# una-auxme/MeshGraphNets.jl

Measured on AMD Instinct MI355X. Metric: processor-step edges/s, higher is better.
Workload: dtype f32; 1 GPU; M-1M jittered-grid triangulation 1000x1000: N=1000000 nodes, E=5992002 directed edges, L=128, hidden_layers=2, 15 processor steps per bench step, fp32 storage, fp16x2 split MFMA (every fp32 operand = two fp16 pieces after a power-of-two scaling per weight chunk / per activation row, three exact piece products per fp32 product on v_mfma_f32_32x32x16_f16), fp32 accumulate; held to the fp32 tolerance; partition=single partition, edge_order=engine re-sorts by receiver once per trajectory (mgn_set_graph)

## Files before the change

meshgraphnets.jl_amd/csrc/kernels.h:

```cpp
#pragma once
#include <hip/hip_runtime.h>
#include <stdint.h>

namespace mgn {

constexpr int TILE = 32;
constexpr int MAX_CHUNKS = 9;

enum { T_B1 = 0, T_B2, T_B3, T_GAMMA, T_BETA, T_BQ, T_LN, T_COUNT };

struct GenMlp {
    const float* chunk[4];
    const float* tabs;
    int32_t nmid;
    int32_t use;
};

struct EdgeArgs {
    const int32_t* snd;
    const int32_t* rcv;
    int64_t E;
    int32_t ntiles;
    const float* P;
    const float* Q;
    float* Elat;
    const float* ElatSrc;
    float* AGG;
    float* CARRY;
    const float* chunk[MAX_CHUNKS];
    const float* chunk_t[MAX_CHUNKS];
    const float* tabs;
    int32_t stagger;
    int32_t tile0;
    unsigned long long* stamps;
    GenMlp gen;
    int32_t c16;
    int32_t bf;
    const uint16_t* split[3];
    const uint16_t* split16[3];
    const uint16_t* splith[3];
    const uint16_t* split16h[3];
    float h2_s[3], h2_rs[3], h2_b2pos;
};

struct NodeArgs {
    int32_t n;
    int32_t ntiles;
    const int32_t* rowptr;
    float* V;
    const float* AGG;
    const float* CARRY;
    float* P;
    float* Q;
    const float* chunk[MAX_CHUNKS];
    const float* chunk_t[MAX_CHUNKS];
    const int32_t* rowptr2; const float* AGG2; const float* CARRY2; int64_t zero_row2;
    const float* tabs;
    int32_t mode;
    int32_t stagger;
    int64_t zero_row;
    int32_t tile0;
    GenMlp gen;
    int32_t c16;
    float* P2; float* Q2; const float* tabs2;
    int32_t bf;
    unsigned long long* stamps;
    const uint16_t* split[7];
    const uint16_t* split16[9];
    const uint16_t* splith[6];
    const uint16_t* split16h[9];
    float h2_s[9], h2_rs[9], h2_b2pos;
};

struct EncNodeArgs {
    int32_t n, ntiles;
    const int32_t* gid;
    const float* srcA; int32_t wa;
    const float* srcB; int32_t wb;
    const float* scale;
    const float* shift;
    const float* w1f;
    float* V; float* P; float* Q;
    const float* chunk[MAX_CHUNKS];
    const float* tabs;
    GenMlp gen;
    const uint16_t* splith[4];
    float h2_rs[4];
};

struct EncEdgeArgs {
    int64_t E; int32_t ntiles;
    const int64_t* gid;
    const float* ef; int32_t Fe;
    const float* scale; const float* shift;
    const float* w1f;
    float* Elat;
    const float* chunk[MAX_CHUNKS];
    const float* tabs;
    GenMlp gen;
    const uint16_t* splith[2];
    float h2_rs[2];
};

struct DecArgs {
    int32_t n, ntiles;
    const float* V;
    const float* w3f;
    const float* b3;
    int32_t O;
    const float* oscale; const float* oshift;
    const float* mask;
    const int32_t* gid;
    float* out;
    const float* chunk[MAX_CHUNKS];
    const float* tabs;
    GenMlp gen;
    const uint16_t* splith[2];
    float h2_rs[2];
};

struct BfEdgeArgs {
    const int32_t* snd; const int32_t* rcv; int64_t E; int32_t ntiles; int32_t tile0;
    const uint16_t* P; const uint16_t* Q;
    uint16_t* Elat; uint16_t* AGG;
    uint16_t* CARRY;
    const uint16_t* chunk[3];
    const float* tabs;
    unsigned long long* stamps;
};
struct BfNodeArgs {
    int32_t n, ntiles; const int32_t* rowptr;
    uint16_t* V; const uint16_t* AGG; const uint16_t* CARRY; uint16_t* P; uint16_t* Q;
    const uint16_t* chunk[7];
    const float* tabs;
    int64_t zero_row; int32_t tile0;
    const int32_t* rowptr2; const uint16_t* AGG2; const uint16_t* CARRY2; int64_t zero_row2;
};
hipError_t launch_edge_bf16(const BfEdgeArgs& a, hipStream_t s);
hipError_t launch_node_bf16(const BfNodeArgs& a, hipStream_t s);
hipError_t launch_project_bf16(const BfNodeArgs& a, hipStream_t s);
hipError_t launch_tile_f32_to_bf16(const float* src, uint16_t* dst, int64_t ntiles, hipStream_t s);
hipError_t launch_tile_bf16_to_f32(const uint16_t* src, float* dst, int64_t ntiles, hipStream_t s);
hipError_t launch_scatter_prows(const float* src, int src_stride , float* dst, int64_t row0, int64_t rows, int L, hipStream_t s);
hipError_t launch_scatter_prows16(const uint16_t* src, int src_stride , uint16_t* dst, int64_t row0, int64_t rows, hipStream_t s);
bool prows_blocked();
hipError_t launch_gather_rows16(const uint16_t* src, const int32_t* idx, uint16_t* dst, int64_t rows, int dst_stride , hipStream_t s);

struct LaunchCfg { int blocks; int threads; size_t lds; };
hipError_t launch_node_split_h(const NodeArgs& a, const LaunchCfg& lc, hipStream_t s);
hipError_t launch_project_split_h(const NodeArgs& a, const LaunchCfg& lc, hipStream_t s);
hipError_t launch_edge_ring_h(const EdgeArgs& a, const LaunchCfg& lc, hipStream_t s);
size_t edge_ring_h_lds();
int set_ringh_stream(int on);
int edge_ring_h_streamed();
hipError_t launch_edge_ring(const EdgeArgs& a, const LaunchCfg& lc, hipStream_t s);
hipError_t launch_node_split(const NodeArgs& a, const LaunchCfg& lc, hipStream_t s);
hipError_t launch_project_split(const NodeArgs& a, const LaunchCfg& lc, hipStream_t s);

struct LinComb {
    int n;
    float c[7];
    const float* k[7];
};
hipError_t launch_lincomb(float* out, const float* u, const LinComb& lc, float dt, int64_t n, hipStream_t s);
hipError_t launch_overwrite(float* x, const float* frame, const uint8_t* mask, int64_t N, int O, hipStream_t s);
int errnorm_partials();
hipError_t launch_errnorm(const float* u, const float* unew, const LinComb& lc, float dt, float atol, float rtol, int64_t n,
                          double* partial, hipStream_t s);
int save_error_blocks(int64_t rows);
hipError_t launch_save_error(const float* x, const float* gt, double* acc, double* part, int64_t N, int O, hipStream_t s);
struct EvalFinish {
    const double* acc;
    const double* part;
    int64_t N; int O, n_saves;
    const int32_t* gid;
    const int64_t* sel;
    int64_t n_val;
    float* mse_time;
    double* mse_save;
    double* vpart;
    int blocks, val_blocks, time_blocks;
};
hipError_t launch_eval_finish(EvalFinish f, hipStream_t s);

bool launch_is_small(int ntiles);
bool node_split_size(int ntiles);
bool launch_is_small_edge(int ntiles_e);
int coop16_enabled();
int set_c16_edge_tiles(int t);
bool ring_hs_default();
bool coop16_size(int ntiles_e, int ntiles_n, bool ring_hs = false);
int last_edge_kernel();
int last_node_kernel();
int set_fp32_split(int on);
int fp32_split_enabled();
int set_split_f16(int on);
int split_f16_enabled();
int set_c16_split(int on);
int c16_split_enabled();
int set_c16_row_tiles(int rt);
int set_kernel_path(int p);
int get_kernel_path();
int set_num_cus(int n);
int num_cus_override();
hipError_t launch_edge_step(int L, const EdgeArgs& a, hipStream_t s);
hipError_t launch_node_step(int L, const NodeArgs& a, hipStream_t s);
hipError_t launch_project(int L, const NodeArgs& a, hipStream_t s);
hipError_t launch_node_project_fused(int L, const NodeArgs& a, hipStream_t s, bool* launched);
hipError_t launch_node_ring_hs(const NodeArgs& a, const LaunchCfg& lc, hipStream_t s);
int node_ring_hs_enabled();
int set_node_ring_hs(int on);
hipError_t launch_enc_node(int L, const EncNodeArgs& a, hipStream_t s);
hipError_t launch_enc_edge(int L, const EncEdgeArgs& a, hipStream_t s);
hipError_t launch_decode(int L, const DecArgs& a, hipStream_t s);
hipError_t launch_gather_rows(const float* src, const int32_t* idx, float* dst, int64_t rows, int L, int dst_stride , hipStream_t s);
hipError_t launch_rows_to_tiles(const float* src, const int64_t* gid64, const int32_t* gid32, float* dst, int64_t rows, int L, hipStream_t s);
hipError_t launch_tiles_to_rows(const float* src, const int64_t* gid64, const int32_t* gid32, float* dst, int64_t rows, int L, hipStream_t s);
hipError_t launch_randn_rows(float* dst, const int64_t* gid64, const int32_t* gid32, int64_t rows, int L,
                             uint64_t seed, hipStream_t s);
int kernels_prow_block();
int split_prow_block();
int checksum_partials();
hipError_t launch_checksum(const float* src, int64_t n, double* partials, hipStream_t s);

}
```

meshgraphnets.jl_amd/csrc/mgn_api.cpp:

```cpp
#include <hip/hip_runtime.h>

#include <algorithm>
#include <cmath>
#include <cstdarg>
#include <cstdint>
#include <cstdio>
#include <cstdlib>
#include <cstring>
#include <ctime>
#include <string>
#include <sys/stat.h>
#include <unistd.h>
#include <vector>

#include "engine_internal.h"
#include "train.h"
#include "graph_dev.h"

using namespace mgn;


namespace {

thread_local std::string g_create_error;
// ... 2146 lines not shown
            if (!write_atomic(ack_of(rank), &rec.nonce, 8)) return fail(h, MGN_E_RCCL, "mgn_comm_init_file: cannot write %s", ack_of(rank).c_str());
            const double t_ack = mtime_of(ack_of(rank));
            for (;;) {
                uint64_t n = 0;
                if (read_exact(go, &n, 8) && mtime_of(go) >= t_ack) {
                    confirmed = n == rec.nonce;
                    break;
                }
                IdFile cur{};
                if (read_exact(base, &cur, sizeof cur) && cur.nonce != rec.nonce) break;
                if (waited > limit) return fail(h, MGN_E_RCCL, "mgn_comm_init_file: timed out waiting for rank 0 to confirm %s", path);
                nap20ms();
                waited += 0.02;
            }
            if (!confirmed) { nap20ms(); waited += 0.02; }
        }
    }
    const int rc = mgn_comm_init(h, rec.id, MGN_COMM_ID_BYTES, transport);
    if (rank == 0) {
        unlink(path);
        unlink(go.c_str());
        for (int r = 1; r < nranks; ++r) unlink(ack_of(r).c_str());
    }
    return rc;
} MGN_CATCH(h)

int mgn_comm_destroy(mgn_handle* h) try {
    if (!h) return MGN_E_ARG;
    if (!h->host_only) (void)hipStreamSynchronize(h->stream);
    delete h->comm;
    h->comm = nullptr;
    h->hx_ready = false;
    h->all_gid.clear();
    return MGN_OK;
} MGN_CATCH(h)

int mgn_comm_barrier(mgn_handle* h) try {
    if (!h) return MGN_E_ARG;
    if (int rc = need_comm(h, "mgn_comm_barrier")) return rc;
    COMMCHK(h, h->comm->barrier(h->stream));
    return MGN_OK;
} MGN_CATCH(h)

int mgn_comm_allreduce(mgn_handle* h, double* x, int32_t n, int32_t op) try {
    if (!h) return MGN_E_ARG;
    if (int rc = need_comm(h, "mgn_comm_allreduce")) return rc;
    if (!x || n < 0 || (op != 0 && op != 1)) return fail(h, MGN_E_ARG, "mgn_comm_allreduce: bad argument");
    COMMCHK(h, h->comm->allreduce_f64(x, n, op, h->stream));
    return MGN_OK;
} MGN_CATCH(h)

int mgn_halo_exchange(mgn_handle* h) try {
    if (int rc = need(h, false, true)) return rc;
    if (int rc = need_comm(h, "mgn_halo_exchange")) return rc;
    if (int rc = exchange_start(h)) return rc;
    return exchange_finish(h);
} MGN_CATCH(h)

int mgn_halo_exchange_host(mgn_handle* h, const float* own_rows, float* halo_rows, int32_t width) try {
    if (!h || !h->have_graph) return fail(h, MGN_E_STATE, "mgn_halo_exchange_host before mgn_set_graph");
    if (int rc = need_comm(h, "mgn_halo_exchange_host")) return rc;
    if (width < 1 || (!own_rows && h->g.n_own) || (!halo_rows && h->g.n_halo)) return fail(h, MGN_E_ARG, "mgn_halo_exchange_host: bad argument");
    const LocalGraph& g = h->g;
    const int P = h->cfg.nranks;
    const size_t rowb = (size_t)width * 4;
    std::vector<float> send(g.send_idx.size() * (size_t)width);
    for (size_t i = 0; i < g.send_idx.size(); ++i) memcpy(send.data() + i * width, own_rows + (size_t)g.send_idx[i] * width, rowb);
    std::vector<size_t> sb(P), so(P), rb(P), ro(P);
    size_t s0 = 0, r0 = 0;
    for (int q = 0; q < P; ++q) {
        sb[q] = (size_t)g.send_rows[q] * rowb; so[q] = s0; s0 += sb[q];
        rb[q] = (size_t)g.recv_rows[q] * rowb; ro[q] = r0; r0 += rb[q];
    }
    COMMCHK(h, h->comm->a2a_host(send.data(), sb.data(), so.data(), halo_rows, rb.data(), ro.data()));
    return MGN_OK;
} MGN_CATCH(h)

int mgn_debug_kernel_path(int path) { return set_kernel_path(path); }
int mgn_debug_c16_row_tiles(int rt) { return set_c16_row_tiles(rt); }
int mgn_debug_c16_edge_tiles(int t) { return set_c16_edge_tiles(t); }
int mgn_debug_fp32_split(int on) { return set_fp32_split(on); }
int mgn_debug_split_f16(int on) { return set_split_f16(on); }
int mgn_debug_ringh_stream(int on) { return set_ringh_stream(on); }
int mgn_debug_node_ring_hs(int on) { return set_node_ring_hs(on); }
int mgn_debug_num_cus(int n) { return set_num_cus(n); }
int mgn_debug_train_f16(int on) { return set_train_f16(on); }
long long mgn_debug_pack_check(mgn_handle* h) try {
    if (int rc = need(h, true, false)) return -rc;
    const int L = h->cfg.L;
    const size_t CH = (size_t)L * L;
    const float* p = h->params.data();
    long long bad = 0;
    std::vector<float> hf(3 * CH), df(3 * CH);
    std::vector<uint16_t> hb(3 * 16384), db(3 * 16384);
    for (const WPackJob& jb : h->wjobs) {
        const float* W = p + jb.src;
        if (jb.kind == 0) {
            const size_t n = (L == 128 ? 3 : 2) * CH;
            pack_chunk(hf.data(), W, jb.ldw, jb.kbase, L);
            pack_chunk_tmajor(hf.data() + CH, hf.data(), L);
            if (L == 128) pack_chunk16(hf.data() + 2 * CH, W, jb.ldw, jb.kbase);
            if (hipMemcpy(df.data(), h->wfrag.as<float>() + jb.off, n * 4, hipMemcpyDeviceToHost) != hipSuccess) return -MGN_E_HIP;
            for (size_t i = 0; i < n; ++i) bad += memcmp(&hf[i], &df[i], 4) != 0;
        } else if (jb.kind == 3) {
            pack_chunk_bf16(hb.data(), W, jb.ldw, jb.kbase);
            if (hipMemcpy(db.data(), h->wbf.as<uint16_t>() + jb.off, 16384 * 2, hipMemcpyDeviceToHost) != hipSuccess) return -MGN_E_HIP;
            for (size_t i = 0; i < 16384; ++i) bad += hb[i] != db[i];
        } else if (jb.kind == 4 || jb.kind == 5) {
            pack_chunk_split_h(hb.data(), W, jb.ldw, jb.kbase, jb.scale, jb.kind == 5);
            if (hipMemcpy(db.data(), h->wsp.as<uint16_t>() + jb.off, 2 * 16384 * 2, hipMemcpyDeviceToHost) != hipSuccess) return -MGN_E_HIP;
            for (size_t i = 0; i < 2 * 16384; ++i) bad += hb[i] != db[i];
        } else {
            pack_chunk_split(hb.data(), W, jb.ldw, jb.kbase, jb.kind == 2);
            if (hipMemcpy(db.data(), h->wsp.as<uint16_t>() + jb.off, 3 * 16384 * 2, hipMemcpyDeviceToHost) != hipSuccess) return -MGN_E_HIP;
            for (size_t i = 0; i < 3 * 16384; ++i) bad += hb[i] != db[i];
        }
    }
    return bad;
} catch (...) { return -MGN_E_OOM; }
int mgn_debug_c16_split(int on) { return set_c16_split(on); }
int mgn_debug_last_node_kernel(void) { return last_node_kernel(); }
int mgn_debug_last_edge_kernel(void) { return last_edge_kernel(); }
int mgn_debug_renumber(int mode) { const int old = g_renumber; g_renumber = mode; return old; }
int mgn_debug_renumbered(const mgn_handle* h) { return h && h->have_graph && h->g.renumbered ? 1 : 0; }

int mgn_debug_edge_stamps(mgn_handle* h, int32_t k, unsigned long long* out ) try {
    if (int rc = need(h, true, true)) return rc;
    const size_t n = 32768;
    HIPCHK(h, h->d_stamps.ensure(n * 8));
    HIPCHK(h, hipMemsetAsync(h->d_stamps.p, 0, n * 8, h->stream));
    if (int rc = mgn_proc_edge(h, k)) return rc;
    HIPCHK(h, hipMemcpyAsync(out, h->d_stamps.p, n * 8, hipMemcpyDeviceToHost, h->stream));
    HIPCHK(h, hipStreamSynchronize(h->stream));
    h->d_stamps.release();
    return MGN_OK;
} MGN_CATCH(h)

int mgn_debug_node_stamps(mgn_handle* h, int32_t k, unsigned long long* out ) try {
    if (int rc = need(h, true, true)) return rc;
    const size_t n = 32768;
    HIPCHK(h, h->d_stamps.ensure(n * 8));
    HIPCHK(h, hipMemsetAsync(h->d_stamps.p, 0, n * 8, h->stream));
    if (int rc = mgn_proc_node(h, k, 1)) return rc;
    HIPCHK(h, hipMemcpyAsync(out, h->d_stamps.p, n * 8, hipMemcpyDeviceToHost, h->stream));
    HIPCHK(h, hipStreamSynchronize(h->stream));
    h->d_stamps.release();
    return MGN_OK;
} MGN_CATCH(h)

int mgn_profile_enable(mgn_handle* h, int32_t on) try {
    if (int rc = need(h, false, false)) return rc;
    HIPCHK(h, hipStreamSynchronize(h->stream));
    for (auto& r : h->recs) {
        h->event_pool.push_back(r.a);
        h->event_pool.push_back(r.b);
    }
    h->recs.clear();
    h->prof = on != 0;
    while (h->prof && h->event_pool.size() < 4096) {
        hipEvent_t e = nullptr;
        if (hipEventCreate(&e) != hipSuccess) break;
        h->event_pool.push_back(e);
    }
    return MGN_OK;
} MGN_CATCH(h)

// ... 25 lines not shown
```

meshgraphnets.jl_amd/csrc/split.hip:

```cpp
#include <cstdlib>

#include "kernels.h"
#include "tile_common.hpp"
#include "split_common.hpp"

namespace mgn {


template <int D> struct SpRing { u32x4 r2[D], r3[D]; };
template <bool G2, bool G3, bool RELU, int D, bool G1 = false, int OFF = 0, bool PRIMED = false, bool NEXT = false>
DEVINL void sp_layer_otf(f32x16 (&acc)[4], const f32x16 (&in)[4], const u32x4* p1, const u32x4* p2, const u32x4* p3, int lane,
                         SpRing<D>* carry = nullptr, const u32x4* nx2 = nullptr, const u32x4* nx3 = nullptr) {
    const u32x4* w1 = p1 + lane;
    const u32x4* w2 = p2 + lane;
    const u32x4* w3 = p3 + lane;
    const N16Buf b1 = n16_buf(G1 ? p1 : nullptr), b2 = n16_buf(G2 ? p2 : nullptr), b3 = n16_buf(G3 ? p3 : nullptr);
    const unsigned voff = (unsigned)lane * 16u;
#define SP_G1(IDX) n16_ldu(b1, voff, (IDX) * 1024)
#define SP_G2(IDX) n16_ldu(b2, voff, (IDX) * 1024)
#define SP_G3(IDX) n16_ldu(b3, voff, (IDX) * 1024)
    static_assert(!(PRIMED || NEXT) || !G1, "ring carry-over is written for the mid / lo streams");
    u32x4 r1[G1 ? D : 1], r2[G2 ? D : 1], r3[G3 ? D : 1];
    if constexpr (PRIMED) {
#pragma unroll
// ... 648 lines not shown
                        acc[t][4 * g + i] = v;
                        sm += v;
                    }
                }
            sm += __shfl_xor(sm, 32, 64);
            const float mean = sm * invL;
            float q = 0.f;
#pragma unroll
            for (int t = 0; t < NT; ++t)
#pragma unroll
                for (int k = 0; k < 16; ++k) {
                    const float d = acc[t][k] - mean;
                    acc[t][k] = d;
                    q += d * d;
                }
            q += __shfl_xor(q, 32, 64);
            const float rstd = ln_rstd_at(q * invL, tb + T_LN * L);
            const f32x4* g4 = reinterpret_cast<const f32x4*>(tb + T_GAMMA * L) + h;
            const f32x4* b4 = reinterpret_cast<const f32x4*>(tb + T_BETA * L) + h;
#pragma unroll
            for (int t = 0; t < NT; ++t) {
#pragma unroll
                for (int g = 0; g < 4; ++g) {
                    const f32x4 gv = g4[2 * (4 * t + g)];
                    const f32x4 bv = b4[2 * (4 * t + g)];
#pragma unroll
                    for (int i = 0; i < 4; ++i) acc[t][4 * g + i] = acc[t][4 * g + i] * rstd * gv[i] + bv[i];
                }
                er[t] += acc[t];
                if (valid) {
#pragma unroll
                    for (int g = 0; g < 4; ++g) {
                        f32x4 v;
#pragma unroll
                        for (int i = 0; i < 4; ++i) v[i] = er[t][4 * g + i];
                        etile[(4 * t + g) * STRIDE_TILE] = v;
                    }
                }
            }
        }
        CST(6);
        EST(2);
        CST(7);
        EST(3);
        const int reff = ix.r >= 0 ? r : (-4 - c);
        const int rprev = __shfl_up(reff, 1, 32);
        const int rnext = __shfl_down(reff, 1, 32);
        const bool head = (c == 0) || (reff != rprev);
        const unsigned hm = (unsigned)__ballot(head);
        const int start = 31 - __clz((int)(hm & (0xFFFFFFFFu >> (31 - c))));
        const int st_in = max(start, c & 16);
        const bool c1 = (c - 1 >= st_in), c2s = (c - 2 >= st_in), c4 = (c - 4 >= st_in), c8 = (c - 8 >= st_in);
        const bool cx = (c >= 16) && (start <= 15);
        EST(4);
        PHASE_FENCE();
        asm volatile("s_nop 1");
        RG_SCAN_LEVEL(acc, c1, "row_shr:1 row_mask:0xf bank_mask:0xf");
        RG_SCAN_LEVEL(acc, c2s, "row_shr:2 row_mask:0xf bank_mask:0xf");
        RG_SCAN_LEVEL(acc, c4, "row_shr:4 row_mask:0xf bank_mask:0xf");
        if (__builtin_amdgcn_ballot_w64(c8) != 0)
        {
            RG_SCAN_LEVEL(acc, c8, "row_shr:8 row_mask:0xf bank_mask:0xf");
        }
        RG_SCAN_LEVEL(acc, cx, "row_bcast:15 row_mask:0xa bank_mask:0xf");
        PHASE_FENCE();
        EST(5);
        const bool tail = valid && ((c == 31) || (reff != rnext));
        const int r_first = __builtin_amdgcn_readfirstlane(reff);
        const bool sl = (start == 0) && (ix.r_before == r_first);
        const bool sr = (c == 31) && (ix.r_after == reff);
        const bool to_carry = sl || sr;
        f32x4* dst = to_carry ? prow_ptr(a.CARRY, (int64_t)2 * tile + (sl ? 0 : 1), L, h) : tile_ptr(a.AGG, r >> 5, L, 32 * h + (r & 31));
        if (tail) store_frag<NT>(dst, to_carry ? STRIDE_PROW : STRIDE_TILE, acc);
        EST(6);
        PHASE_FENCE();
        load_frag<NT>(acc, prow_ptr(a.Q, ixn.r >= 0 ? ixn.r : 0, L, h), STRIDE_PROW);
        EST(7);
        ix = ixn;
        tw.tile += tw.stride;
    }
}

constexpr int HS_W = 4;
#define MGN_HS_REQ_STEP 0
#define MGN_HS_AHEAD 4
template <int NCH>
struct RsT {
    static constexpr int W = HS_W;
    static constexpr int WPL = 32 / W;
    static constexpr int NW = NCH * WPL;
    static constexpr int NB = 3;
    static constexpr int BUF = 2 * W * 64;
    static constexpr int AHEAD = MGN_HS_AHEAD;
    static constexpr int SLOTS = AHEAD - 1;
    static_assert(NW % NB == 0 && NW % SLOTS == 0 && AHEAD >= 3, "static window -> buffer / slot mapping");
};
typedef RsT<3> Rs;
template <int LYR>
DEVINL RhFrag rs_first(const u32x4* ring) {
    constexpr int b = (Rs::WPL * LYR) % Rs::NB;
    RhFrag f;
    f.h = ring[b * Rs::BUF];
    f.l = ring[b * Rs::BUF + 64];
    return f;
}
template <int NCH>
struct RsSrcT {
    const u32x4* w[NCH];
};
typedef RsSrcT<3> RsSrc;
DEVINL const u32x4* rs_src(const u32x4* chunk, int w, int e) { return chunk + ((e >> 6) & 1) * 2048 + (w * Rs::W + (e >> 7)) * 64 + (e & 63); }
template <int LYR, int FIN, int RFS = 0, int NWV = 8, bool WRAP = false, int NCH = 3, bool PREMUL = false>
DEVINL void hs_layer_ring(f32x16 (&acc)[4], f32x16 (&in)[4], u32x4* ring, const RsSrcT<NCH>& src, RhFrag& nx, u32x4 (&pend)[Rs::SLOTS][Rs::BUF / (NWV * 64)], int lane,
                          int tid, float sx, float cfin = 0.f, const float* btab = nullptr, const f32x4* rf = nullptr, const N16Buf* rfb = nullptr, int rfs_rt = 0, float premul = 1.f) {
    constexpr int ROT = 2;
    constexpr int W = Rs::W, WPL = Rs::WPL, NW = RsT<NCH>::NW, BUF = Rs::BUF, NB = Rs::NB;
    constexpr int LPT = BUF / (NWV * 64);
    f32x4 side[2 * ROT];
    if constexpr (!WRAP && RFS > 0) {
#pragma unroll
        for (int m = 0; m < 2 * ROT; ++m) side[m] = rf[m * RFS];
    }
    auto bias = [&](int sn, int u) {
        f32x2 b = {0.f, 0.f};
        if constexpr (FIN == 2) b = *reinterpret_cast<const f32x2*>(btab + 8 * (4 * (sn >> 1) + 2 * (sn & 1) + (u >> 1)) + 2 * (u & 1));
        return b;
    };
    unsigned ph[4], pl[4];
#pragma unroll
    for (int u = 0; u < 4; ++u) {
        const f32x2 b = bias(0, u);
        h2_split_pair<FIN>(ph[u], pl[u], in[0][2 * u], in[0][2 * u + 1], sx, cfin, b[0], b[1]);
    }
    unsigned voff[LPT];
#pragma unroll
    for (int i = 0; i < LPT; ++i) {
        const int e = i * NWV * 64 + tid;
        voff[i] = (unsigned)((((e >> 6) & 1) * 2048 + (e >> 7) * 64 + (e & 63)) * 16);
        asm volatile("" : "+v"(voff[i]));
    }
    __builtin_amdgcn_sched_barrier(0);
#pragma unroll
    for (int s = 0; s < 8; ++s) {
        unsigned nh[4], nl[4];
#pragma unroll
        for (int t = 0; t < 4; ++t) {
            const int it = 4 * s + t;
            const int gw = WPL * LYR + it / W;
            const u32x4 a1 = nx.h, a2 = nx.l;
            if (it % W == MGN_HS_REQ_STEP) {
                const int g2 = (gw + Rs::AHEAD) % NW, l2 = g2 / WPL, w2 = g2 % WPL;
#pragma unroll
                for (int i = 0; i < LPT; ++i)
                    pend[gw % Rs::SLOTS][i] = *reinterpret_cast<const u32x4*>(reinterpret_cast<const char*>(src.w[l2] + w2 * W * 64) + voff[i]);
            }
            if constexpr (RFS != 0) {
                if ((t & 1) && s < 8 - ROT) {
                    f32x4 v;
                    if constexpr (WRAP && RFS < 0) v = rf[(int64_t)(2 * s + (t >> 1)) * rfs_rt];
                    else if constexpr (WRAP) v = n16_ld(*rfb, (unsigned)lane * 16u, (2 * s + (t >> 1)) * 1024);
                    else v = rf[(2 * (s + ROT) + (t >> 1)) * RFS];
#pragma unroll
                    for (int i = 0; i < 4; ++i) in[s >> 1][8 * (s & 1) + 4 * (t >> 1) + i] = v[i];
                }
            }
            if (it + 1 < 32) {
// ... 140 lines not shown
        hs_layer_ring<1, 1, 0, NWV>(y, acc, ring, src, nx, pend, lane, tid, x2.s);
        CST(3);
        const float c2 = x2.rs * rsw2;
        const H2Scale x3 = h2_scale(__builtin_fmaf(h2_rowmax<false>(y), c2, b2pos));
        zero_frag<NT>(acc);
        CST(4);
        const N16Buf enb = n16_buf(a.Elat + (int64_t)nxt * (TILE * L), TILE * L * 4);
        hs_layer_ring<2, 2, STRIDE_TILE, NWV, true>(acc, y, ring, src, nx, pend, lane, tid, x3.s, c2, tb + T_B2 * L + 4 * h, nullptr, &enb);
        CST(5);
        EST(1);
        PHASE_FENCE();
        __builtin_amdgcn_s_setprio(MGN_PRIO);
#pragma unroll
        for (int m = 12; m < 16; ++m) {
            const f32x4 v = n16_ld(enb, (unsigned)lane * 16u, m * 1024);
#pragma unroll
            for (int i = 0; i < 4; ++i) y[3][4 * (m & 3) + i] = v[i];
        }
        {
            constexpr float invL = 1.0f / 128;
            const float c3 = x3.rs * rsw3;
            const f32x4* b34 = reinterpret_cast<const f32x4*>(tb + T_B3 * L) + h;
            float sm = 0.f;
#pragma unroll
            for (int t = 0; t < NT; ++t)
#pragma unroll
                for (int g = 0; g < 4; ++g) {
                    const f32x4 bv = b34[2 * (4 * t + g)];
#pragma unroll
                    for (int i = 0; i < 4; ++i) {
                        const float v = __builtin_fmaf(acc[t][4 * g + i], c3, bv[i]);
                        acc[t][4 * g + i] = v;
                        sm += v;
                    }
                }
            sm += __shfl_xor(sm, 32, 64);
            const float mean = sm * invL;
            float q = 0.f;
#pragma unroll
            for (int t = 0; t < NT; ++t)
#pragma unroll
                for (int k = 0; k < 16; ++k) {
                    const float d = acc[t][k] - mean;
                    acc[t][k] = d;
                    q += d * d;
                }
            q += __shfl_xor(q, 32, 64);
            const float rstd = ln_rstd_at(q * invL, tb + T_LN * L);
            const f32x4* g4 = reinterpret_cast<const f32x4*>(tb + T_GAMMA * L) + h;
            const f32x4* b4 = reinterpret_cast<const f32x4*>(tb + T_BETA * L) + h;
#pragma unroll
            for (int t = 0; t < NT; ++t) {
#pragma unroll
                for (int g = 0; g < 4; ++g) {
                    const f32x4 gv = g4[2 * (4 * t + g)];
                    const f32x4 bv = b4[2 * (4 * t + g)];
#pragma unroll
                    for (int i = 0; i < 4; ++i) acc[t][4 * g + i] = acc[t][4 * g + i] * rstd * gv[i] + bv[i];
                }
#pragma unroll
                for (int g = 0; g < 4; ++g) {
                    f32x4 v = park[(4 * t + g) * 64 + lane];
#pragma unroll
                    for (int i = 0; i < 4; ++i) v[i] += acc[t][4 * g + i];
                    if (valid) etile[(4 * t + g) * STRIDE_TILE] = v;
                }
            }
        }
        CST(6);
        EST(2);
        CST(7);
        EST(3);
        const int reff = ix.r >= 0 ? r : (-4 - c);
        const int rprev = __shfl_up(reff, 1, 32);
        const int rnext = __shfl_down(reff, 1, 32);
        const bool head = (c == 0) || (reff != rprev);
        const unsigned hm = (unsigned)__ballot(head);
        const int start = 31 - __clz((int)(hm & (0xFFFFFFFFu >> (31 - c))));
        const int st_in = max(start, c & 16);
        const bool c1 = (c - 1 >= st_in), c2s = (c - 2 >= st_in), c4 = (c - 4 >= st_in), c8 = (c - 8 >= st_in);
        const bool cx = (c >= 16) && (start <= 15);
        EST(4);
        PHASE_FENCE();
        asm volatile("s_nop 1");
        RG_SCAN_LEVEL(acc, c1, "row_shr:1 row_mask:0xf bank_mask:0xf");
        RG_SCAN_LEVEL(acc, c2s, "row_shr:2 row_mask:0xf bank_mask:0xf");
        RG_SCAN_LEVEL(acc, c4, "row_shr:4 row_mask:0xf bank_mask:0xf");
        if (__builtin_amdgcn_ballot_w64(c8) != 0)
        {
            RG_SCAN_LEVEL(acc, c8, "row_shr:8 row_mask:0xf bank_mask:0xf");
        }
        RG_SCAN_LEVEL(acc, cx, "row_bcast:15 row_mask:0xa bank_mask:0xf");
        PHASE_FENCE();
        EST(5);
        const bool tail = valid && ((c == 31) || (reff != rnext));
        const int r_first = __builtin_amdgcn_readfirstlane(reff);
        const bool sl = (start == 0) && (ix.r_before == r_first);
        const bool sr = (c == 31) && (ix.r_after == reff);
        const bool to_carry = sl || sr;
        f32x4* dst = to_carry ? prow_ptr(a.CARRY, (int64_t)2 * tile + (sl ? 0 : 1), L, h) : tile_ptr(a.AGG, r >> 5, L, 32 * h + (r & 31));
        if (tail) store_frag<NT>(dst, to_carry ? STRIDE_PROW : STRIDE_TILE, acc);
        EST(6);
        PHASE_FENCE();
        load_frag<NT>(acc, prow_ptr(a.Q, ixn.r >= 0 ? ixn.r : 0, L, h), STRIDE_PROW);
        EST(7);
        ix = ixn;
        tw.tile += tw.stride;
    }
}


#define MGN_NODE_MPRIO MGN_PRIO
#define MGN_SP2_D3 4
template <bool TWO>
__global__ __launch_bounds__(512, 2) void k_node_split(const NodeArgs a) {
    constexpr int NT = 4, L = 128, PC = 16384, D = MGN_SP2_D;
    extern __shared__ __attribute__((aligned(16))) float smem[];
    uint16_t* wl = reinterpret_cast<uint16_t*>(smem);
    {
        const bool fast = a.ntiles <= MGN_FAST_PRELOAD_TILES;
        copy_to_lds16(wl, a.split[2], PC, fast);
        copy_to_lds16(wl + PC, a.split[3], PC, fast);
        copy_to_lds16(wl + 2 * PC, a.split[0], PC, fast);
        copy_to_lds16(wl + 3 * PC, a.split[1], PC, fast);
    }
    float* tb = smem + 4 * PC / 2;
    copy_to_lds(tb, a.tabs, T_COUNT * L);
    __syncthreads();
    const u32x4* lvh = reinterpret_cast<const u32x4*>(wl);
    const u32x4* lah = reinterpret_cast<const u32x4*>(wl + PC);
    const u32x4* l2h = reinterpret_cast<const u32x4*>(wl + 2 * PC);
    const u32x4* l3h = reinterpret_cast<const u32x4*>(wl + 3 * PC);
    const u32x4* gv = reinterpret_cast<const u32x4*>(a.split[2]);
    const u32x4* ga = reinterpret_cast<const u32x4*>(a.split[3]);
    const u32x4* g2 = reinterpret_cast<const u32x4*>(a.split[0]);
    const u32x4* g3 = reinterpret_cast<const u32x4*>(a.split[1]);
    const int lane0 = threadIdx.x & 63;
    const int wave = __builtin_amdgcn_readfirstlane(threadIdx.x >> 6);
    stagger_second_half(wave, a.stagger);
    TileWalk tw(a.ntiles, wave, MGN_SPREAD_ROUNDS_NODE);
    if (tw.tile >= tw.end) return;
    f32x16 x[NT], acc[NT];
    load_frag<NT>(x, tile_ptr(a.V, tw.tile, L, lane0), STRIDE_TILE);
    for (;;) {
        OPAQUE_LANE();
        const int tile = tw.tile;
        const int next = tile + tw.stride;
        const bool has_next = next < tw.end;
        const int n = tile * TILE + c;
        const bool valid = n < a.n;
        const int nn = valid ? n : 0;
        f32x4* vtile = tile_ptr(a.V, tile, L, lane);
        __builtin_amdgcn_s_setprio(0);
        tab_frag<NT>(acc, tb + T_B1 * L, h);
        constexpr int O1 = 32 % D, O2 = 64 % D, O3 = 96 % D;
        SpRing<D> rg;
        sp_layer_otf<true, true, false, D, false, 0, false, true>(acc, x, lvh, gv + 2048, gv + 4096, lane, &rg, ga + 2048, ga + 4096);
        LOAD_AGGREGATE(NT, x, a.rowptr, a.AGG, a.CARRY, a.zero_row);
        if constexpr (TWO) {
            sp_layer_otf<true, true, false, D, false, O1, true, false>(acc, x, lah, ga + 2048, ga + 4096, lane, &rg);
            const u32x4* gb = reinterpret_cast<const u32x4*>(a.split[6]);
            LOAD_AGGREGATE(NT, x, a.rowptr2, a.AGG2, a.CARRY2, a.zero_row2);
            sp_layer_otf<true, true, false, MGN_SP2_D3, true>(acc, x, gb, gb + 2048, gb + 4096, lane);
            tab_frag<NT>(x, tb + T_B2 * L, h);
            sp_layer_otf<true, true, true, D, false, 0, false, true>(x, acc, l2h, g2 + 2048, g2 + 4096, lane, &rg, g3 + 2048, g3 + 4096);
            tab_frag<NT>(acc, tb + T_B3 * L, h);
            sp_layer_otf<true, true, true, D, false, O1, true, false>(acc, x, l3h, g3 + 2048, g3 + 4096, lane, &rg);
        } else {
            sp_layer_otf<true, true, false, D, false, O1, true, true>(acc, x, lah, ga + 2048, ga + 4096, lane, &rg, g2 + 2048, g2 + 4096);
            tab_frag<NT>(x, tb + T_B2 * L, h);
            sp_layer_otf<true, true, true, D, false, O2, true, true>(x, acc, l2h, g2 + 2048, g2 + 4096, lane, &rg, g3 + 2048, g3 + 4096);
            tab_frag<NT>(acc, tb + T_B3 * L, h);
            sp_layer_otf<true, true, true, D, false, O3, true, false>(acc, x, l3h, g3 + 2048, g3 + 4096, lane, &rg);
        }
        PHASE_FENCE();
        __builtin_amdgcn_s_setprio(MGN_NODE_MPRIO);
        load_frag<NT>(x, vtile, STRIDE_TILE);
        layer_norm_frag<NT>(acc, tb + T_GAMMA * L, tb + T_BETA * L, h);
#pragma unroll
        for (int t = 0; t < NT; ++t) x[t] += acc[t];
        if (valid) store_frag<NT>(vtile, STRIDE_TILE, x);
        if (!has_next) break;
        PHASE_FENCE();
        load_frag<NT>(x, tile_ptr(a.V, next, L, lane), STRIDE_TILE);
        tw.tile = next;
    }
}
// ... 246 lines not shown
#pragma unroll
            for (int i = 0; i < 4; ++i) x[3][4 * (m & 3) + i] = v[i];
        }
        {
            const int n1 = nxt * TILE + c;
            ra0 = n1 < a.n ? a.rowptr[n1] : 0;
            ra1 = n1 < a.n ? a.rowptr[n1 + 1] : 0;
        }
        h2_finish_frag<NT>(acc, sp.rs * rswq, tb + T_BQ * L, h);
        if (valid) store_frag<NT>(prow_ptr(a.Q, nn, L, h), STRIDE_PROW, acc);
        tw.tile += tw.stride;
    }
}

__global__ __launch_bounds__(512, 2) void k_project_split_h(const NodeArgs a) {
    constexpr int NT = 4, L = 128, PC = 16384;
    extern __shared__ __attribute__((aligned(16))) float smem[];
    uint16_t* wl = reinterpret_cast<uint16_t*>(smem);
    {
        const bool fast = a.ntiles <= MGN_FAST_PRELOAD_TILES;
        copy_to_lds16(wl, a.splith[4], 2 * PC, fast);
        copy_to_lds16(wl + 2 * PC, a.splith[5], 2 * PC, fast);
    }
    float* tb = smem + 4 * PC / 2;
    copy_to_lds(tb, a.tabs, T_COUNT * L);
    __syncthreads();
    const u32x4* lph = reinterpret_cast<const u32x4*>(wl);
    const u32x4* lpl = reinterpret_cast<const u32x4*>(wl + PC);
    const u32x4* lqh = reinterpret_cast<const u32x4*>(wl + 2 * PC);
    const u32x4* lql = reinterpret_cast<const u32x4*>(wl + 3 * PC);
    const float rswp = a.h2_rs[4], rswq = a.h2_rs[5];
    const int lane0 = threadIdx.x & 63;
    const int wave = __builtin_amdgcn_readfirstlane(threadIdx.x >> 6);
    TileWalk tw(a.ntiles, wave, MGN_SPREAD_ROUNDS_NODE);
    if (tw.tile >= tw.end) return;
    f32x16 x[NT], acc[NT];
    load_frag<NT>(x, tile_ptr(a.V, a.tile0 + tw.tile, L, lane0), STRIDE_TILE);
    for (;;) {
        OPAQUE_LANE();
        const int tile = a.tile0 + tw.tile;
        const int next = tw.tile + tw.stride;
        const bool has_next = next < tw.end;
        const int n = tile * TILE + c;
        const bool valid = n < a.n;
        const int nn = valid ? n : 0;
        __builtin_amdgcn_s_setprio(0);
        const H2Scale sv = h2_scale(h2_rowmax<true>(x));
        zero_frag<NT>(acc);
        h2_layer_otf<false, 0, 1>(acc, x, lph, lpl, lane, sv.s);
        __builtin_amdgcn_s_setprio(MGN_NODE_MPRIO);
        h2_scale_frag<NT>(acc, sv.rs * rswp);
        if (valid) store_frag<NT>(prow_ptr(a.P, nn, L, h), STRIDE_PROW, acc);
        __builtin_amdgcn_s_setprio(0);
        zero_frag<NT>(acc);
        h2_layer_otf<false, 0, 1>(acc, x, lqh, lql, lane, sv.s);
        __builtin_amdgcn_s_setprio(MGN_NODE_MPRIO);
        h2_finish_frag<NT>(acc, sv.rs * rswq, tb + T_BQ * L, h);
        if (valid) store_frag<NT>(prow_ptr(a.Q, nn, L, h), STRIDE_PROW, acc);
        if (!has_next) break;
        PHASE_FENCE();
        load_frag<NT>(x, tile_ptr(a.V, a.tile0 + next, L, lane), STRIDE_TILE);
        tw.tile = next;
    }
}

template <typename K, typename A>
static hipError_t sp_launch(K kern, const A& a, const LaunchCfg& lc, hipStream_t s, bool& attr_set) {
    if (!attr_set) {
        const hipError_t e = hipFuncSetAttribute(reinterpret_cast<const void*>(kern), hipFuncAttributeMaxDynamicSharedMemorySize, 160 * 1024);
        if (e != hipSuccess) return e;
        attr_set = true;
    }
    hipLaunchKernelGGL(kern, dim3(lc.blocks), dim3(lc.threads), lc.lds, s, a);
    return hipGetLastError();
}
hipError_t launch_edge_ring(const EdgeArgs& a, const LaunchCfg& lc, hipStream_t s) {
    static bool attr_set8 = false, attr_set4 = false;
    if (lc.threads == 256) return sp_launch(k_edge_ring<4>, a, lc, s, attr_set4);
    return sp_launch(k_edge_ring<8>, a, lc, s, attr_set8);
}
static int g_ringh_stream = [] { const char* e = getenv("MGN_RINGH_STREAM"); return e ? atoi(e) : 1; }();
int edge_ring_h_streamed() { return g_ringh_stream; }
int set_ringh_stream(int on) { const int old = g_ringh_stream; g_ringh_stream = on; return old; }
hipError_t launch_edge_ring_h(const EdgeArgs& a, const LaunchCfg& lc, hipStream_t s) {
    static bool attr_set8 = false, attr_set4 = false, attr_s8 = false, attr_s4 = false;
    if (g_ringh_stream) {
        LaunchCfg ls = lc;
        ls.lds = (size_t)Rs::NB * Rs::BUF * 16 + (size_t)(lc.threads / 64) * 16384 + (size_t)T_COUNT * 128 * 4 + 64;
        if (lc.threads == 256) return sp_launch(k_edge_ring_hs<4>, a, ls, s, attr_s4);
        return sp_launch(k_edge_ring_hs<8>, a, ls, s, attr_s8);
    }
    if (lc.threads == 256) return sp_launch(k_edge_ring_h<4>, a, lc, s, attr_set4);
    return sp_launch(k_edge_ring_h<8>, a, lc, s, attr_set8);
}
size_t edge_ring_h_lds() { return (size_t)3 * 32768 + (size_t)Rh<MGN_RINGH_W>::NB * Rh<MGN_RINGH_W>::BUF * 16 + (size_t)T_COUNT * 128 * 4 + 64; }
hipError_t launch_node_split(const NodeArgs& a, const LaunchCfg& lc, hipStream_t s) {
    static bool attr_set = false;
    static bool attr_set2 = false;
    if (a.AGG2) return sp_launch(k_node_split<true>, a, lc, s, attr_set2);
    return sp_launch(k_node_split<false>, a, lc, s, attr_set);
}
hipError_t launch_node_split_h(const NodeArgs& a, const LaunchCfg& lc, hipStream_t s) {
    static bool attr_set = false;
    return sp_launch(k_node_split_h, a, lc, s, attr_set);
}
static int g_node_ring_hs = [] { const char* e = getenv("MGN_NODE_RING_HS"); return e ? atoi(e) : 1; }();
int node_ring_hs_enabled() { return g_node_ring_hs; }
int set_node_ring_hs(int on) { const int old = g_node_ring_hs; g_node_ring_hs = on; return old; }
hipError_t launch_node_ring_hs(const NodeArgs& a, const LaunchCfg& lc, hipStream_t s) {
    static bool attr_set = false;
    LaunchCfg ls = lc;
    ls.threads = 512;
    ls.lds = (size_t)Rs::NB * Rs::BUF * 16 + (size_t)8 * 16384 + (size_t)T_COUNT * 128 * 4 + 64;
    return sp_launch(k_node_ring_hs, a, ls, s, attr_set);
}
hipError_t launch_project_split_h(const NodeArgs& a, const LaunchCfg& lc, hipStream_t s) {
    static bool attr_set = false;
    return sp_launch(k_project_split_h, a, lc, s, attr_set);
}
hipError_t launch_project_split(const NodeArgs& a, const LaunchCfg& lc, hipStream_t s) {
    static bool attr_set = false;
    return sp_launch(k_project_split, a, lc, s, attr_set);
}

int split_prow_block() { return MGN_PROW_BLOCK; }

}
```

Baseline: 2.001 billion edges/s.

## Pack per-receiver Q loads and AGG stores through LDS staging in edge ring

In the streamed edge ring kernel, each 32-edge tile's distinct receivers are compacted with ballot/popc. When there are few distinct receivers, the Q rows are loaded once per unique receiver and broadcast through an LDS staging area instead of one row load per edge. An optional mode (off by default) likewise compacts tail stores to AGG/CARRY through LDS so each lane writes packed destinations. This cuts redundant global traffic for receiver-sorted edges, at the cost of extra permutes, readlanes, LDS round trips and fences, plus higher register pressure from prefetching HS_QI Q fragments early.

```diff
diff --git a/meshgraphnets.jl_amd/csrc/kernels.h b/meshgraphnets.jl_amd/csrc/kernels.h
--- a/meshgraphnets.jl_amd/csrc/kernels.h
+++ b/meshgraphnets.jl_amd/csrc/kernels.h
@@ -41,6 +41,7 @@
     const uint16_t* splith[3];
     const uint16_t* split16h[3];
     float h2_s[3], h2_rs[3], h2_b2pos;
+    int32_t recv_pack;
 };
 
 struct NodeArgs {
@@ -152,6 +153,7 @@
 hipError_t launch_edge_ring_h(const EdgeArgs& a, const LaunchCfg& lc, hipStream_t s);
 size_t edge_ring_h_lds();
 int set_ringh_stream(int on);
+int set_ring_recv_pack(int bits);
 int edge_ring_h_streamed();
 hipError_t launch_edge_ring(const EdgeArgs& a, const LaunchCfg& lc, hipStream_t s);
 hipError_t launch_node_split(const NodeArgs& a, const LaunchCfg& lc, hipStream_t s);
diff --git a/meshgraphnets.jl_amd/csrc/mgn_api.cpp b/meshgraphnets.jl_amd/csrc/mgn_api.cpp
--- a/meshgraphnets.jl_amd/csrc/mgn_api.cpp
+++ b/meshgraphnets.jl_amd/csrc/mgn_api.cpp
@@ -2252,6 +2252,7 @@
 int mgn_debug_fp32_split(int on) { return set_fp32_split(on); }
 int mgn_debug_split_f16(int on) { return set_split_f16(on); }
 int mgn_debug_ringh_stream(int on) { return set_ringh_stream(on); }
+int mgn_debug_ring_recv_pack(int bits) { return set_ring_recv_pack(bits); }
 int mgn_debug_node_ring_hs(int on) { return set_node_ring_hs(on); }
 int mgn_debug_num_cus(int n) { return set_num_cus(n); }
 int mgn_debug_train_f16(int on) { return set_train_f16(on); }
diff --git a/meshgraphnets.jl_amd/csrc/split.hip b/meshgraphnets.jl_amd/csrc/split.hip
--- a/meshgraphnets.jl_amd/csrc/split.hip
+++ b/meshgraphnets.jl_amd/csrc/split.hip
@@ -754,6 +754,12 @@
 }
 
 constexpr int HS_W = 4;
+constexpr int HS_AI = 8;
+#ifndef MGN_HS_QI
+#define MGN_HS_QI 4
+#endif
+constexpr int HS_QI = MGN_HS_QI;      static_assert(HS_QI >= 1 && HS_QI <= 8, "packed Q loads");
+constexpr int HS_SS = 34;
 #define MGN_HS_REQ_STEP 0
 #define MGN_HS_AHEAD 4
 template <int NCH>
@@ -1060,6 +1066,22 @@
         const bool cx = (c >= 16) && (start <= 15);
         EST(4);
         PHASE_FENCE();
+        const int rn = ixn.r;
+        const bool headn = (c == 0) || (rn != __shfl_up(rn, 1, 32));
+        const unsigned hmn = (unsigned)__ballot(headn);
+        const int slotn = __popc(hmn & (0xFFFFFFFFu >> (31 - c))) - 1;
+        const int nrn = __popc(hmn);
+        const bool packq = (a.recv_pack & 2) && nrn <= 2 * HS_QI;
+        const int rows = __builtin_amdgcn_ds_permute(4 * ((headn && h == 0) ? slotn : 32 + c), rn >= 0 ? rn : 0);
+        f32x4 qv[HS_QI];
+#pragma unroll
+        for (int k = 0; k < HS_QI; ++k) {
+            const int r0 = __builtin_amdgcn_readlane(rows, min(2 * k, nrn - 1)), r1 = __builtin_amdgcn_readlane(rows, min(2 * k + 1, nrn - 1));
+            const unsigned row = packq ? (unsigned)(h ? r1 : r0) : (unsigned)(rn >= 0 ? rn : 0);
+            const int off = packq ? (lane & 1) + ((lane >> 1) & 15) * STRIDE_PROW : h + k * STRIDE_PROW;
+            qv[k] = (reinterpret_cast<const f32x4*>(a.Q) + prow_index((int64_t)row, L))[off];
+        }
+        PHASE_FENCE();
         asm volatile("s_nop 1");
         RG_SCAN_LEVEL(acc, c1, "row_shr:1 row_mask:0xf bank_mask:0xf");
         RG_SCAN_LEVEL(acc, c2s, "row_shr:2 row_mask:0xf bank_mask:0xf");
@@ -1076,11 +1098,59 @@
         const bool sl = (start == 0) && (ix.r_before == r_first);
         const bool sr = (c == 31) && (ix.r_after == reff);
         const bool to_carry = sl || sr;
-        f32x4* dst = to_carry ? prow_ptr(a.CARRY, (int64_t)2 * tile + (sl ? 0 : 1), L, h) : tile_ptr(a.AGG, r >> 5, L, 32 * h + (r & 31));
-        if (tail) store_frag<NT>(dst, to_carry ? STRIDE_PROW : STRIDE_TILE, acc);
+        f32x4* stg = park;
+        const unsigned tm = (unsigned)__ballot(tail);
+        const int nrecv = __popc(tm);
+        if ((a.recv_pack & 1) && nrecv <= 2 * HS_AI) {
+            const int slot = __popc(tm & ((1u << c) - 1u));
+            const f32x4* d0 = to_carry ? prow_ptr(a.CARRY, (int64_t)2 * tile + (sl ? 0 : 1), L, 0) : tile_ptr(a.AGG, r >> 5, L, r & 31);
+            const uint64_t dq = reinterpret_cast<uint64_t>(d0) | (to_carry ? 1u : 0u);
+            const int push = 4 * ((tail && h == 0) ? slot : 32 + c);
+            const int dlo = __builtin_amdgcn_ds_permute(push, (int)(unsigned)dq), dhi = __builtin_amdgcn_ds_permute(push, (int)(unsigned)(dq >> 32));
+            if (tail) store_frag<NT>(stg + slot * HS_SS + h, 2, acc);
+            __builtin_amdgcn_fence(__ATOMIC_ACQ_REL, "wavefront");
+            const int pm = (lane >> 1) & 15, ph = lane & 1;
+            const unsigned off_agg = (unsigned)(32 * ph + pm * STRIDE_TILE) * 16u, off_carry = (unsigned)(ph + pm * STRIDE_PROW) * 16u;
+#pragma unroll
+            for (int g = 0; g < HS_AI / 4; ++g)
+                if (8 * g < nrecv) {
+                    f32x4 v[4];
+#pragma unroll
+                    for (int j = 0; j < 4; ++j) v[j] = stg[min(8 * g + 2 * j + h, nrecv - 1) * HS_SS + (lane & 31)];
+#pragma unroll
+                    for (int j = 0; j < 4; ++j) {
+                        const int k = 4 * g + j;
+                        if (2 * k < nrecv) {
+                            const int s0 = 2 * k, s1 = min(2 * k + 1, nrecv - 1);
+                            const unsigned lo = (unsigned)(h ? __builtin_amdgcn_readlane(dlo, s1) : __builtin_amdgcn_readlane(dlo, s0));
+                            const unsigned hi = (unsigned)(h ? __builtin_amdgcn_readlane(dhi, s1) : __builtin_amdgcn_readlane(dhi, s0));
+                            const uint64_t q = ((uint64_t)hi << 32) | (lo & ~1u);
+                            *reinterpret_cast<f32x4*>(q + ((lo & 1u) ? off_carry : off_agg)) = v[j];
+                        }
+                    }
+                }
+        } else {
+            f32x4* dst = to_carry ? prow_ptr(a.CARRY, (int64_t)2 * tile + (sl ? 0 : 1), L, h) : tile_ptr(a.AGG, r >> 5, L, 32 * h + (r & 31));
+            if (tail) store_frag<NT>(dst, to_carry ? STRIDE_PROW : STRIDE_TILE, acc);
+        }
         EST(6);
         PHASE_FENCE();
-        load_frag<NT>(acc, prow_ptr(a.Q, ixn.r >= 0 ? ixn.r : 0, L, h), STRIDE_PROW);
+        if (packq) {
+            __builtin_amdgcn_fence(__ATOMIC_ACQ_REL, "wavefront");
+#pragma unroll
+            for (int k = 0; k < HS_QI; ++k) stg[(2 * k + h) * HS_SS + (lane & 31)] = qv[k];
+            __builtin_amdgcn_fence(__ATOMIC_ACQ_REL, "wavefront");
+            load_frag<NT>(acc, stg + slotn * HS_SS + h, 2);
+            __builtin_amdgcn_fence(__ATOMIC_ACQ_REL, "wavefront");
+        } else {
+            const f32x4* qrow = prow_ptr(a.Q, ixn.r >= 0 ? ixn.r : 0, L, h);
+#pragma unroll
+            for (int m = 0; m < 16; ++m) {
+                const f32x4 v = m < HS_QI ? qv[m] : qrow[m * STRIDE_PROW];
+#pragma unroll
+                for (int i = 0; i < 4; ++i) acc[m >> 2][4 * (m & 3) + i] = v[i];
+            }
+        }
         EST(7);
         ix = ixn;
         tw.tile += tw.stride;
@@ -1493,13 +1563,20 @@
 static int g_ringh_stream = [] { const char* e = getenv("MGN_RINGH_STREAM"); return e ? atoi(e) : 1; }();
 int edge_ring_h_streamed() { return g_ringh_stream; }
 int set_ringh_stream(int on) { const int old = g_ringh_stream; g_ringh_stream = on; return old; }
+#ifndef MGN_RING_RECV_PACK
+#define MGN_RING_RECV_PACK 2
+#endif
+static int g_ring_recv_pack = MGN_RING_RECV_PACK;
+int set_ring_recv_pack(int bits) { const int old = g_ring_recv_pack; g_ring_recv_pack = bits & 3; return old; }
 hipError_t launch_edge_ring_h(const EdgeArgs& a, const LaunchCfg& lc, hipStream_t s) {
     static bool attr_set8 = false, attr_set4 = false, attr_s8 = false, attr_s4 = false;
     if (g_ringh_stream) {
         LaunchCfg ls = lc;
         ls.lds = (size_t)Rs::NB * Rs::BUF * 16 + (size_t)(lc.threads / 64) * 16384 + (size_t)T_COUNT * 128 * 4 + 64;
-        if (lc.threads == 256) return sp_launch(k_edge_ring_hs<4>, a, ls, s, attr_s4);
-        return sp_launch(k_edge_ring_hs<8>, a, ls, s, attr_s8);
+        EdgeArgs ap = a;
+        ap.recv_pack = g_ring_recv_pack;
+        if (lc.threads == 256) return sp_launch(k_edge_ring_hs<4>, ap, ls, s, attr_s4);
+        return sp_launch(k_edge_ring_hs<8>, ap, ls, s, attr_s8);
     }
     if (lc.threads == 256) return sp_launch(k_edge_ring_h<4>, a, lc, s, attr_set4);
     return sp_launch(k_edge_ring_h<8>, a, lc, s, attr_set8);
```

Result: no change. 2.003 billion edges/s, median of 2 (+0.1%).
